# joyce-leesw/Conway-s-GOL-Distributed

Hardware: AMD Instinct MI355X
Metric: cell updates/sec (GCUPS) at 16384² & 65536², 1/2/4/8 MI355X; % HBM roofline (higher is better)
Workload: dtype u32

## Files before the change

### conway-s-gol-distributed_amd/csrc/gol_tile.h

```cpp
#pragma once
#include "gol_device.h"
#if GOL_TOOLS
#include "gol_tile_turn.h"
#else
namespace golk {
template <int SEG, int V>
__device__ __forceinline__ void tile_turn_asm(uint32_t (&v)[SEG][2], uint32_t (&ad)[4], uint32_t ps,
                                              uint32_t ba);
}
#endif

#include <type_traits>

#ifndef GOL_TILE_PAIRS_MAX
#define GOL_TILE_PAIRS_MAX 12
#endif
#ifndef GOL_TURN_VAR
#define GOL_TURN_VAR 4
#endif
#ifndef GOL_TILE_WEST_CARRY
#define GOL_TILE_WEST_CARRY 1
#endif
#ifndef GOL_TILE_RAW
#define GOL_TILE_RAW 0
#endif
#ifndef GOL_TILE_PAIR
#define GOL_TILE_PAIR 0
#endif
#ifndef GOL_TILE_SPIN_LIMIT
#define GOL_TILE_SPIN_LIMIT (1 << 22)
#endif
template <int SEG, int W>
constexpr bool tile_west_carry() { return GOL_TILE_WEST_CARRY && W == 1 && SEG >= 4 && SEG <= 16; }

namespace golk {

constexpr int kTileMaxWaves = 16;
constexpr size_t tile_lds_bytes(int threads, int words)
{
    return (size_t)threads * 4 * 16 * words + 4 * kTileMaxWaves;
}
constexpr int tile_seg_rows(int code) { return code % 100; }
constexpr int tile_seg_words(int code) { return code / 1000 + 1; }
constexpr int tile_slots_pow2(int threads)
{
    int n = 64;
    while (n < threads) n *= 2;
    return n;
}
constexpr size_t tile_count_lds_bytes(int threads)
{
    return 4 * (size_t)kMaxTileTurns * kTileMaxWaves + 4 * (size_t)threads;
}
constexpr size_t tile_lds_bytes_code(int threads, int code)
{
    const int ord = code / 100 % 10;
    return (ord == 8 || ord == 9) && (GOL_TURN_VAR & 4)
               ? tile_lds_bytes(tile_slots_pow2(threads), 1)
           : ord == 3 && GOL_TILE_PAIR ? 2 * tile_lds_bytes(threads, 1)
                                       : tile_lds_bytes(threads, tile_seg_words(code));
}

constexpr uint32_t tile_rcp16(int c) { return (65536u + (uint32_t)c - 1u) / (uint32_t)c; }
constexpr bool tile_rcp16_exact()
{
    for (int c = 3; c <= 64; ++c)
        for (uint32_t l = 0; l < 64; ++l)
            if (((l * tile_rcp16(c)) >> 16) != l / (uint32_t)c) return false;
    return true;
}
static_assert(tile_rcp16_exact(), "lane * ceil(65536 / C) >> 16 == lane / C below 64");

struct TilePos {
    int tw, th, x0, y0, g;
    uint32_t rcp;
};
__device__ __forceinline__ TilePos tile_pos_rect(const StepArgs &a, int tile, int ntx)
{
    const int ty = tile / ntx, tx = tile - ty * ntx;
    const int c = a.tile_w + 2;
    return TilePos{a.tile_w, a.band, tx * a.tile_w, a.row_lo + ty * a.band, 64 / c, tile_rcp16(c)};
}
struct TileLaunch {
    int ntiles, n_main, ntx_main;
    uint32_t inv_ntx;
    int narrow_w, narrow_h;
    int g[2];
    uint32_t rcp[2];
};
__device__ __forceinline__ TilePos tile_pos(const StepArgs &a, const TileLaunch &L, int tile)
{
    if (tile >= L.n_main)
        return TilePos{L.narrow_w, L.narrow_h, L.ntx_main * a.tile_w,
                       a.row_lo + (tile - L.n_main) * L.narrow_h, L.g[1], L.rcp[1]};
    int ty = tile;
    if (L.ntx_main > 1) {
        ty = (int)__umulhi((uint32_t)tile, L.inv_ntx);
        ty -= ty * L.ntx_main > tile ? 1 : 0;
    }
    const int tx = tile - ty * L.ntx_main;
    return TilePos{a.tile_w, a.band, tx * a.tile_w, a.row_lo + ty * a.band, L.g[0], L.rcp[0]};
}

struct RingArgs {
    int tile, ntx;
    uint64_t *u0, *u1;
    unsigned *flags;
    unsigned epoch;
    int turns;
    unsigned *gcount;
    unsigned gbase;
    int ablate;
};
template <int SEG, int ORD, int W, bool PERSIST, bool RING = false, bool CNT = false,
          bool SEAM = false, bool BIG = false>
__device__ __forceinline__ void tile_pass(const uint64_t *__restrict__ in,
                                          uint64_t *__restrict__ out, const StepArgs &a,
                                          int turns, const TilePos &pos,
                                          RingArgs ra = RingArgs{})
{
    constexpr int ND = 2 * W;
    constexpr int NS = 2 * ND;
    static_assert(SEG >= 2, "two edge rows per segment");
    extern __shared__ uint4 xsh[];
    const int nslot = (int)(blockDim.x);
    const int TW = pos.tw, C = TW + 2, G = pos.g;
    const int K = turns, TH = pos.th;
    const int nl = a.nw / W;
    const int y0 = pos.y0;
    const int x0 = pos.x0;
    const int lane = threadIdx.x & 63;
    const int wave = __builtin_amdgcn_readfirstlane((int)(threadIdx.x >> 6));
    const int group = (int)(((uint32_t)lane * pos.rcp) >> 16), col = lane - group * C;
    const bool live = group < G;
    const int nseg = (TH + 2 * K + SEG - 1) / SEG;
    constexpr bool kHalo = ORD == 7;
    static_assert(!kHalo || W == 1, "ORD 7: one word per lane");
    const int seg = !kHalo ? wave * G + group
                           : wave == 0 ? (group == 0 ? 0 : nseg - 1) : (wave - 1) * G + group + 1;
    const bool rev = kHalo && wave == 0 && group == 1;
    const int slot = seg * C + col;

    int gx = x0 - 1 + (live ? col : 0);
    if (nl < C) {
        while (gx < 0) gx += nl;
        while (gx >= nl) gx -= nl;
    } else {
        gx += gx < 0 ? nl : 0;
        gx -= gx >= nl ? nl : 0;
    }
    static_assert(!SEAM || (W == 1 && !PERSIST && !RING && !CNT && ORD != 3 && ORD < 7),
                  "seam launches: plain k_step_tile, one word per lane, no counts");
    [[maybe_unused]] bool seam_tile = false, seam_lane = false;
    [[maybe_unused]] int seam_v = 0;
    [[maybe_unused]] uint32_t seam_d = 0;
    if constexpr (SEAM) {
        const int L = nl - 1;
        seam_tile = x0 == 0 || x0 + TW >= L;
        seam_v = x0 - 1 + (live ? col : 0);
        seam_lane = seam_tile && live && (seam_v < 0 || seam_v >= L);
        const int g2 = seam_lane ? min(seam_second_col(seam_v, L), L) : gx;
        seam_d = (uint32_t)(g2 - gx) * 8u;
    }
    const int M = a.modrows;
    const uint32_t pitch_b = (uint32_t)a.pitch * 8u;
    const uint32_t span = (uint32_t)M * pitch_b;
    int rbase = y0 - K;
    if (rbase < 0) {
        rbase += M;
        while (rbase < 0) rbase += M;
    }
    int r = rbase + (live ? seg : 0) * SEG + (rev ? SEG - 1 : 0);
    if (__builtin_amdgcn_ballot_w64(r >= 2 * M) != 0) {
        while (r >= M) r -= M;
    } else {
        r -= r >= M ? M : 0;
    }
    uint32_t off = (uint32_t)r * pitch_b + (uint32_t)gx * (8u * W);
    [[maybe_unused]] const uint32_t off_first = off;
    const uint32_t lstep = rev ? span - pitch_b : pitch_b;
    const __amdgpu_buffer_rsrc_t rin =
        __builtin_amdgcn_make_buffer_rsrc((void *)in, (short)0, (int)span, kBufFlags);
    static_assert(!BIG || (W == 1 && !PERSIST && !RING && !CNT && !SEAM && ORD != 3 && ORD < 7),
                  "big launches: plain k_step_tile, one word per lane, no seam, no counts");
    [[maybe_unused]] int big_ra = 0, big_rb = 0, big_rs = 0;
    [[maybe_unused]] __amdgpu_buffer_rsrc_t rin_a = rin, rin_b = rin;
    [[maybe_unused]] auto big_rsrc = [](const void *p, uint64_t byte, int rows, uint32_t row_b) {
        const uint64_t ad = (uint64_t)(uintptr_t)p + byte;
        const uint32_t lo = (uint32_t)__builtin_amdgcn_readfirstlane((int)(uint32_t)ad);
        const uint32_t hi = (uint32_t)__builtin_amdgcn_readfirstlane((int)(uint32_t)(ad >> 32));
        const int bytes = __builtin_amdgcn_readfirstlane((int)((uint32_t)rows * row_b));
        return __builtin_amdgcn_make_buffer_rsrc((void *)(uintptr_t)(((uint64_t)hi << 32) | lo),
                                                 (short)0, bytes, kBufFlags);
    };
    if constexpr (BIG) {
        int64_t w0, wa, wb;
        uint64_t ba;
        (void)tile_window(M, a.pitch, y0, K, TH, &w0, &wa, &wb, &ba);
        big_ra = __builtin_amdgcn_readfirstlane((int)wa);
        big_rb = __builtin_amdgcn_readfirstlane((int)wb);
        big_rs = big_ra > 0 ? max(0, min(TH, a.row_hi - y0)) : 0;
        rin_a = big_rsrc(in, ba, big_ra, pitch_b);
        rin_b = big_rsrc(in, 0, big_rb, pitch_b);
    }
    const __amdgpu_buffer_rsrc_t rout =
        BIG ? big_rsrc(out, (uint64_t)(uint32_t)y0 * pitch_b, big_rs, pitch_b)
            : __builtin_amdgcn_make_buffer_rsrc((void *)out, (short)0, (int)span, kBufFlags);

    constexpr int kLoadAux = PERSIST ? 16 : GOL_TILE_LOAD_AUX;
    uint32_t v[SEG][ND];
    auto load_row = [&](int i, uint32_t voff, uint32_t soff) {
        if constexpr (W == 1) {
            const u32x2 w = __builtin_amdgcn_raw_buffer_load_b64(rin, voff, soff, kLoadAux);
            v[i][0] = w.x;
            v[i][1] = w.y;
        } else {
            const u32x4 w = __builtin_amdgcn_raw_buffer_load_b128(rin, voff, soff, kLoadAux);
            v[i][0] = w.x;
            v[i][1] = w.y;
            v[i][2] = w.z;
            v[i][3] = w.w;
        }
    };
    if constexpr (BIG) {
        const int tr0 = (live ? seg : 0) * SEG;
        const uint32_t cb = (uint32_t)gx * 8u;
        const int wlim = big_ra + big_rb;
        if (__builtin_amdgcn_ballot_w64(tr0 + SEG > big_ra) == 0) {
            const uint32_t o = (uint32_t)tr0 * pitch_b + cb;
#pragma unroll
            for (int i = 0; i < SEG; ++i) {
                const u32x2 w = __builtin_amdgcn_raw_buffer_load_b64(rin_a, o, (uint32_t)i * pitch_b, kLoadAux);
                v[i][0] = w.x;
                v[i][1] = w.y;
            }
        } else if (big_rb == 0) {
#pragma unroll
            for (int i = 0; i < SEG; ++i) {
                const uint32_t o = (uint32_t)min(tr0 + i, wlim) * pitch_b + cb;
                const u32x2 w = __builtin_amdgcn_raw_buffer_load_b64(rin_a, o, 0, kLoadAux);
                v[i][0] = w.x;
                v[i][1] = w.y;
            }
        } else {
            constexpr int kBigChunk = 4;
            int tb = tr0;
#pragma unroll
            for (int c0 = 0; c0 < SEG; c0 += kBigChunk) {
                u32x2 pa[kBigChunk], pb[kBigChunk];
#pragma unroll
                for (int j = 0; j < kBigChunk; ++j) {
                    if (c0 + j < SEG) {
                        const int t = min(tb + c0 + j, wlim);
                        const uint32_t oa = (uint32_t)t * pitch_b + cb;
                        const uint32_t ob = (uint32_t)(t - big_ra) * pitch_b + cb;
                        pa[j] = __builtin_amdgcn_raw_buffer_load_b64(rin_a, oa, 0, kLoadAux);
                        pb[j] = __builtin_amdgcn_raw_buffer_load_b64(rin_b, ob, 0, kLoadAux);
                    }
                }
#pragma unroll
                for (int j = 0; j < kBigChunk; ++j) {
                    if (c0 + j < SEG) {
                        const bool second = tb + c0 + j >= big_ra;
                        v[c0 + j][0] = second ? pb[j].x : pa[j].x;
                        v[c0 + j][1] = second ? pb[j].y : pa[j].y;
                    }
                }
                if (c0 + kBigChunk < SEG)
                    asm volatile("" : "+v"(tb) : "v"(v[c0 + kBigChunk - 1][0]),
                                 "v"(v[c0 + kBigChunk - 1][1]));
            }
        }
    } else if (SEAM && seam_tile) {
    } else if (!kHalo && __builtin_amdgcn_ballot_w64(r + SEG > M) == 0) {
#pragma unroll
        for (int i = 0; i < SEG; ++i) load_row(i, off, (uint32_t)i * pitch_b);
    } else {
#pragma unroll
        for (int i = 0; i < SEG; ++i) {
            load_row(i, off, 0);
            off += lstep;
            off = off >= span ? off - span : off;
        }
    }
    if constexpr (SEAM) {
        if (seam_tile) {
            const int L = nl - 1, rb = a.width & 63;
            auto seam_load = [&](auto ODD, auto STEP) {
                constexpr bool odd = decltype(ODD)::value, step = decltype(STEP)::value;
                constexpr int kSeamChunk = 4;
                uint32_t o1 = off_first, o2 = off_first + seam_d;
#pragma unroll
                for (int c0 = 0; c0 < SEG; c0 += kSeamChunk) {
                    u32x2 p[kSeamChunk], t[kSeamChunk];
#pragma unroll
                    for (int j = 0; j < kSeamChunk; ++j) {
                        if (c0 + j < SEG) {
                            const uint32_t so = step ? (uint32_t)(c0 + j) * pitch_b : 0u;
                            p[j] = __builtin_amdgcn_raw_buffer_load_b64(rin, o1, so, kLoadAux);
                            t[j] = __builtin_amdgcn_raw_buffer_load_b64(rin, o2, so, kLoadAux);
                            if constexpr (!step) {
                                o1 += lstep;
                                o1 = o1 >= span ? o1 - span : o1;
                                o2 += lstep;
                                o2 = o2 >= span ? o2 - span : o2;
                            }
                        }
                    }
#pragma unroll
                    for (int j = 0; j < kSeamChunk; ++j) {
                        if (c0 + j < SEG) {
                            const uint64_t pw = ((uint64_t)p[j].y << 32) | p[j].x;
                            const uint64_t sw = ((uint64_t)t[j].y << 32) | t[j].x;
                            const uint64_t w = seam_stitch(pw, sw, seam_v, L, rb, odd, true);
                            v[c0 + j][0] = seam_lane ? (uint32_t)w : p[j].x;
                            v[c0 + j][1] = seam_lane ? (uint32_t)(w >> 32) : p[j].y;
                        }
                    }
                    if (c0 + kSeamChunk < SEG)
                        asm volatile("" : "+v"(o1), "+v"(o2) : "v"(v[c0 + kSeamChunk - 1][0]),
                                     "v"(v[c0 + kSeamChunk - 1][1]));
                }
            };
            using std::false_type;
            using std::true_type;
            const bool nowrap = __builtin_amdgcn_ballot_w64(r + SEG > M) == 0;
            if (rb & 1) {
                if (nowrap) seam_load(true_type{}, true_type{});
                else seam_load(true_type{}, false_type{});
            } else {
                if (nowrap) seam_load(false_type{}, true_type{});
                else seam_load(false_type{}, false_type{});
            }
        }
    }

    auto rsum = [&](const uint32_t (&x)[ND], uint32_t (&s)[NS]) {
        const uint32_t Rt = dpp_from_upper_z(x[0]);
#pragma unroll
        for (int w = 0; w < W; ++w) {
            const uint32_t e = x[2 * w], o = x[2 * w + 1];
            uint32_t wl;
            if constexpr (tile_west_carry<SEG, W>()) {
                const uint64_t m = __builtin_amdgcn_ballot_w64((int)o < 0) << 1;
                uint64_t co;
                asm("v_addc_co_u32_e64 %0, %1, %2, %2, %3" : "=v"(wl), "=&s"(co) : "v"(o), "s"(m));
            } else {
                const uint32_t L = dpp_from_lower_z(x[ND - 1]);
                wl = __builtin_amdgcn_alignbit(o, w == 0 ? L : x[2 * w - 1], 31);
            }
            const uint32_t er = __builtin_amdgcn_alignbit(w == W - 1 ? Rt : x[2 * w + 2], e, 1);
            s[4 * w + 0] = xor3(wl, e, o);
            s[4 * w + 1] = maj(wl, e, o);
            s[4 * w + 2] = xor3(e, o, er);
            s[4 * w + 3] = maj(e, o, er);
        }
    };
    auto rule = [&](const uint32_t (&A)[NS], const uint32_t (&B)[NS], const uint32_t (&Cs)[NS],
                   uint32_t (&x)[ND]) {
        uint32_t n[ND];
#pragma unroll
        for (int d = 0; d < ND; ++d)
            n[d] = life_rule7(A[2 * d], B[2 * d], Cs[2 * d], A[2 * d + 1], B[2 * d + 1],
                              Cs[2 * d + 1], x[d]);
#pragma unroll
        for (int d = 0; d < ND; ++d) x[d] = n[d];
    };
    auto put = [&](uint4 *base, const uint32_t (&S)[NS]) {
#pragma unroll
        for (int q = 0; q < W; ++q)
            base[(size_t)q * nslot * 4] =
                make_uint4(S[4 * q], S[4 * q + 1], S[4 * q + 2], S[4 * q + 3]);
    };
    auto get = [&](const uint4 *base, uint32_t (&S)[NS]) {
#pragma unroll
        for (int q = 0; q < W; ++q) {
            const uint4 u = base[(size_t)q * nslot * 4];
            S[4 * q] = u.x;
            S[4 * q + 1] = u.y;
            S[4 * q + 2] = u.z;
            S[4 * q + 3] = u.w;
        }
    };
    const int nlive = (int)(blockDim.x >> 6) * G * C;
    const int myslot = live ? slot : nlive + wave * (64 - G * C) + (lane - G * C);
    const int s_up = live && seg > 0 ? slot - C : myslot;
    const int s_dn = live && seg + 1 < nseg ? slot + C : myslot;
    const int o_wt = (rev ? (int)nslot : 0) + myslot, o_wb = (rev ? 0 : (int)nslot) + myslot;
    const int o_up = rev ? s_dn : (int)nslot + s_up, o_dn = rev ? (int)nslot + s_up : s_dn;
    constexpr bool kPairs = SEG * W <= GOL_TILE_PAIRS_MAX;
    constexpr bool kRaw = ORD < 4 && W == 1 && SEG <= GOL_TILE_RAW;
    uint4 *const wtop2[2] = {xsh + o_wt, xsh + 2 * nslot + o_wt};
    uint4 *const wbot2[2] = {xsh + o_wb, xsh + 2 * nslot + o_wb};
    const uint4 *const rup2[2] = {xsh + o_up, xsh + 2 * nslot + o_up};
    const uint4 *const rdn2[2] = {xsh + o_dn, xsh + 2 * nslot + o_dn};
    auto wtop = [&](int p, int off) { return kPairs ? wtop2[p] : xsh + off + o_wt; };
    auto wbot = [&](int p, int off) { return kPairs ? wbot2[p] : xsh + off + o_wb; };
    auto rup = [&](int p, int off) { return kPairs ? rup2[p] : (const uint4 *)(xsh + off + o_up); };
    auto rdn = [&](int p, int off) { return kPairs ? rdn2[p] : (const uint4 *)(xsh + off + o_dn); };
    const int wrow0 = __builtin_amdgcn_readfirstlane(
        !kHalo ? wave * G * SEG : wave == 0 ? 0 : ((wave - 1) * G + 1) * SEG);
    const int wrow1 = __builtin_amdgcn_readfirstlane(
        !kHalo ? wrow0 + G * SEG : wave == 0 ? 1 << 30 : wrow0 + G * SEG);
    const int nwaves = (int)(blockDim.x >> 6);
    volatile int *const flag = (volatile int *)(xsh + 4 * (size_t)nslot * W);
    if constexpr (ORD == 4) {
        if (lane == 0) flag[wave] = -1;
        __syncthreads();
    }
    static_assert(!CNT || (W == 1 && !PERSIST && !RING && ORD != 3 && ORD < 7),
                  "counted launches: plain k_step_tile, one word per lane");
    [[maybe_unused]] uint32_t *const csum = (uint32_t *)(xsh + 4 * (size_t)nslot * W) + kTileMaxWaves;
    [[maybe_unused]] int cw_lo = 0, cw_hi = -1;
    static_assert(!CNT || SEG <= 32, "counted launches: one word of row bits per lane");
    [[maybe_unused]] bool cwave = false, cuni = false, cany = false;
    [[maybe_unused]] uint32_t *const crow = csum + kMaxTileTurns * kTileMaxWaves;
    if constexpr (CNT) {
        cw_lo = K / (G * SEG);
        cw_hi = min(nwaves - 1, (K + TH - 1) / (G * SEG));
        cwave = wave >= cw_lo && wave <= cw_hi;
        const int ybase = y0 - K + seg * SEG;
        const int ylo = max(y0, a.cnt_lo), yhi = min(min(y0 + TH, a.row_hi), a.cnt_hi);
        const bool ccol = live && col >= 1 && col <= TW && x0 + col - 1 < nl;
        const int ci_lo = min(max(ylo - ybase, 0), SEG), ci_hi = min(max(yhi - ybase, 0), SEG);
        const int cn = ccol && cwave ? max(ci_hi - ci_lo, 0) : 0;
        crow[threadIdx.x] = cn > 0 ? (~0u >> (32 - cn)) << ci_lo : 0u;
        cany = cn > 0;
        cuni = __builtin_amdgcn_ballot_w64(cn != 0 && cn != SEG) == 0;
    }
    auto bcnt = [](uint32_t x, uint32_t acc) {
        uint32_t r;
        asm("v_bcnt_u32_b32 %0, %1, %2" : "=v"(r) : "v"(x), "v"(acc));
        return r;
    };
    auto bcnt0 = [](uint32_t x) {
        uint32_t r;
        asm("v_bcnt_u32_b32 %0, %1, 0" : "=v"(r) : "v"(x));
        return r;
    };
    auto count_turn = [&](int t) {
        if constexpr (CNT) {
            if (!cwave) return;
            uint32_t acc;
            if (cuni) {
                acc = bcnt(v[0][1], bcnt0(v[0][0]));
#pragma unroll
                for (int i = 1; i < SEG; ++i) acc = bcnt(v[i][1], bcnt(v[i][0], acc));
                acc = cany ? acc : 0u;
            } else {
                uint32_t all = ~0u;
                asm volatile("" : "+v"(all));
                const uint32_t ln = __builtin_amdgcn_mbcnt_hi(all, __builtin_amdgcn_mbcnt_lo(all, 0u));
                const uint32_t rlo = crow[wave * 64 + (int)ln];
                acc = 0;
#pragma unroll
                for (int i = 0; i < SEG; ++i) {
                    const uint32_t m = 0u - ((rlo >> i) & 1u);
                    acc = bcnt(v[i][1] & m, bcnt(v[i][0] & m, acc));
                }
                asm("s_nop 1" : "+v"(acc));
            }
            acc += (uint32_t)__builtin_amdgcn_update_dpp(0, (int)acc, 0x111, 0xf, 0xf, true);
            acc += (uint32_t)__builtin_amdgcn_update_dpp(0, (int)acc, 0x112, 0xf, 0xf, true);
            acc += (uint32_t)__builtin_amdgcn_update_dpp(0, (int)acc, 0x114, 0xf, 0xf, true);
            acc += (uint32_t)__builtin_amdgcn_update_dpp(0, (int)acc, 0x118, 0xf, 0xf, true);
            acc += (uint32_t)__builtin_amdgcn_update_dpp(0, (int)acc, 0x142, 0xa, 0xf, false);
            acc += (uint32_t)__builtin_amdgcn_update_dpp(0, (int)acc, 0x143, 0xc, 0xf, false);
            if (lane == 63) csum[t * kTileMaxWaves + wave] = acc;
        }
    };
    auto publish = [&](int t) {
        if constexpr (ORD == 4) {
            asm volatile("" ::: "memory");
            if (lane == 0) flag[wave] = t;
        }
    };
    auto await_neighbours = [&](int t) {
        if constexpr (ORD == 4) {
            const int up = wave > 0 ? wave - 1 : wave, dn = wave + 1 < nwaves ? wave + 1 : wave;
            for (;;) {
                const int a = __builtin_amdgcn_readfirstlane(flag[up]);
                const int b = __builtin_amdgcn_readfirstlane(flag[dn]);
                if (a >= t && b >= t) break;
                __builtin_amdgcn_s_sleep(1);
            }
            __builtin_amdgcn_fence(__ATOMIC_ACQUIRE, "workgroup");
        }
    };
    auto turn4 = [&](auto P, int poff, int t, int lo_rt) {
        constexpr int p = decltype(P)::value;
        const int lo = ORD == 7 ? lo_rt : 0;
        const int off = poff;
        uint32_t Pw[NS], Q[NS], S1[NS];
        {
            uint32_t F[NS], Lr[NS];
            rsum(v[0], F);
            rsum(v[SEG - 1], Lr);
            put(wtop(p, off), F);
            put(wbot(p, off), Lr);
            if constexpr (ORD == 5 || ORD == 7) __syncthreads();
            else if constexpr (ORD == 4) publish(t);
#pragma unroll
            for (int k = 0; k < NS; ++k) Pw[k] = F[k];
        }
        rsum(v[1], Q);
#pragma unroll
        for (int k = 0; k < NS; ++k) S1[k] = Q[k];
#pragma unroll
        for (int i = 1; i + 1 < SEG; ++i) {
            uint32_t R[NS];
            if (i + 2 == SEG) get(wbot(p, off), R);
            else rsum(v[i + 1], R);
            if (i >= lo) rule(Pw, Q, R, v[i]);
#pragma unroll
            for (int k = 0; k < NS; ++k) {
                Pw[k] = Q[k];
                Q[k] = R[k];
            }
        }
#pragma unroll
        for (int i = 1; i + 1 < SEG; ++i)
#pragma unroll
            for (int d = 0; d < ND; ++d) asm volatile("" : "+v"(v[i][d]));
        if constexpr (ORD == 6) __syncthreads();
        else await_neighbours(t);
        uint32_t U[NS], D[NS], F[NS];
        if (lo == 0) {
            get(rup(p, off), U);
            get(wtop(p, off), F);
            rule(U, F, S1, v[0]);
        }
        get(rdn(p, off), D);
        get(wbot(p, off), F);
        rule(Pw, F, D, v[SEG - 1]);
    };
    auto turn = [&](auto P, int poff, int t) {
        if constexpr (ORD >= 4) {
            turn4(P, poff, t, kHalo && wave == 0 ? min(t + 1, SEG - 2) : 0);
            return;
        }
        constexpr int p = decltype(P)::value;
        const int off = poff;
        uint32_t F[NS], Lr[NS];
        rsum(v[0], F);
        rsum(v[SEG - 1], Lr);
        if constexpr (kRaw) {
            *wtop(p, off) = make_uint4(v[0][0], v[0][1], v[SEG - 1][0], v[SEG - 1][1]);
        } else {
            put(wtop(p, off), F);
            put(wbot(p, off), Lr);
        }
        uint32_t U[NS], D[NS];
        auto get_raw = [&](uint32_t (&Us)[NS], uint32_t (&Ds)[NS]) {
            const uint4 *const base = kPairs ? xsh + 2 * nslot * p : xsh + off;
            const uint2 a = *(reinterpret_cast<const uint2 *>(base + s_up) + 1);
            const uint2 b = *reinterpret_cast<const uint2 *>(base + s_dn);
            const uint32_t ra[ND] = {a.x, a.y}, rb[ND] = {b.x, b.y};
            rsum(ra, Us);
            rsum(rb, Ds);
        };
        if constexpr (ORD < 2 || ORD == 3) {
            if constexpr (ORD != 3) __syncthreads();
            if constexpr (kRaw) {
                get_raw(U, D);
            } else {
                get(rup(p, off), U);
                get(rdn(p, off), D);
            }
        }
        if constexpr (ORD == 0 || ORD == 3) {
            uint32_t A[NS], B[NS];
#pragma unroll
            for (int k = 0; k < NS; ++k) {
                A[k] = U[k];
                B[k] = F[k];
            }
#pragma unroll
            for (int i = 0; i < SEG; ++i) {
                uint32_t Cs[NS];
                if (i + 1 == SEG) {
#pragma unroll
                    for (int k = 0; k < NS; ++k) Cs[k] = D[k];
                } else if (i + 2 == SEG) {
#pragma unroll
                    for (int k = 0; k < NS; ++k) Cs[k] = Lr[k];
                } else {
                    rsum(v[i + 1], Cs);
                }
                rule(A, B, Cs, v[i]);
#pragma unroll
                for (int k = 0; k < NS; ++k) {
                    A[k] = B[k];
                    B[k] = Cs[k];
                }
            }
        } else {
            uint32_t Pw[NS], Q[NS], S1[NS];
#pragma unroll
            for (int k = 0; k < NS; ++k) Pw[k] = F[k];
            if constexpr (SEG >= 3) {
                rsum(v[1], Q);
#pragma unroll
                for (int k = 0; k < NS; ++k) S1[k] = Q[k];
            } else {
#pragma unroll
                for (int k = 0; k < NS; ++k) S1[k] = Q[k] = Lr[k];
            }
#pragma unroll
            for (int i = 1; i + 1 < SEG; ++i) {
                uint32_t R[NS];
                if (i + 2 == SEG) {
#pragma unroll
                    for (int k = 0; k < NS; ++k) R[k] = Lr[k];
                } else {
                    rsum(v[i + 1], R);
                }
                rule(Pw, Q, R, v[i]);
#pragma unroll
                for (int k = 0; k < NS; ++k) {
                    Pw[k] = Q[k];
                    Q[k] = R[k];
                }
            }
            if constexpr (ORD == 2) {
                __syncthreads();
                if constexpr (kRaw) {
                    get_raw(U, D);
                } else {
                    get(rup(p, off), U);
                    get(rdn(p, off), D);
                }
            }
            rule(U, F, S1, v[0]);
            rule(Pw, Lr, D, v[SEG - 1]);
        }
    };
    const int lastrow = 2 * K + TH - 1;
    auto leave = [&](int t) {
        if constexpr (ORD == 4) {
            if (lane == 0) flag[wave] = 0x7fffffff;
        }
    };
    bool gone = false;
    if constexpr (RING) {
        static_assert(PERSIST && W == 1 && ORD != 4 && ORD != 7 && ORD < 8, "K1r: one word per lane");
        const int THv = min(TH, a.row_hi - y0), TWv = min(TW, nl - x0);
        const int nty = (a.row_hi - a.row_lo + TH - 1) / TH;
        const int tile = ra.tile, ntx = ra.ntx, ty = tile / ntx, tx = tile - ty * ntx;
        const int nblocks = (ra.turns + K - 1) / K, kbase = ra.turns / nblocks,
                  kextra = ra.turns % nblocks;
        bool gave_up = false;
        for (int b = 0; b < nblocks; ++b) {
            const int kb = kbase + (b < kextra ? 1 : 0);
            if constexpr (!kPairs) {
                for (int t = 0; t < kb; ++t) turn(std::integral_constant<int, 0>{}, (t & 1) * 2 * nslot, t);
            } else {
                for (int t = 0; t < kb; t += 2) {
                    turn(std::integral_constant<int, 0>{}, 0, t);
                    if (t + 1 == kb) break;
                    turn(std::integral_constant<int, 1>{}, 0, t + 1);
                }
            }
            if (b + 1 == nblocks) break;
            uint64_t *const X = (b & 1) ? ra.u1 : ra.u0;
            const __amdgpu_buffer_rsrc_t rx =
                __builtin_amdgcn_make_buffer_rsrc((void *)X, (short)0, (int)span, kBufFlags);
            int ln = lane, thv = THv, twv = TWv, kk = K;
            uint32_t off0 = off_first;
            asm volatile("" : "+v"(ln), "+v"(off0), "+s"(thv), "+s"(twv), "+s"(kk));
            const int gr = (int)(((uint32_t)ln * pos.rcp) >> 16), cl = ln - gr * C;
            const bool lv = gr < G;
            const int tr0 = (wave * G + gr) * SEG;
            if (lv && cl >= 1 && cl <= twv && !(ra.ablate & 1)) {
                const bool side = cl == 1 || cl == twv;
                uint32_t so = off0;
#pragma unroll
                for (int i = 0; i < SEG; ++i) {
                    const int j = tr0 + i - kk;
                    if (j >= 0 && j < thv && (side || j < kk || j >= thv - kk))
                        buf_store(v[i], rx, so, 0);
                    so += pitch_b;
                    so = so >= span ? so - span : so;
                }
            }
            __builtin_amdgcn_s_waitcnt((7 << 4) | (15 << 8));
            __syncthreads();
            if (threadIdx.x == 0) {
                __hip_atomic_store(ra.flags + tile, ra.epoch + (unsigned)b + 1u, __ATOMIC_RELAXED,
                                   __HIP_MEMORY_SCOPE_AGENT);
            }
            if (ra.gcount && threadIdx.x == 0) {
                __hip_atomic_fetch_add(ra.gcount, 1u, __ATOMIC_RELAXED, __HIP_MEMORY_SCOPE_AGENT);
                const unsigned want = ra.gbase + (unsigned)(b + 1) * (unsigned)(nty * ntx);
                bool seen = false;
                for (int spin = 0; !seen && spin < GOL_TILE_SPIN_LIMIT; ++spin) {
                    const unsigned fv = __hip_atomic_load(ra.gcount, __ATOMIC_RELAXED, __HIP_MEMORY_SCOPE_AGENT);
                    seen = (int)(fv - want) >= 0;
                    if (!seen) __builtin_amdgcn_s_sleep(1);
                }
                gave_up |= !seen;
            }
            if (!ra.gcount && threadIdx.x < 8 && !(ra.ablate & 2)) {
                const int jn = (int)threadIdx.x + (threadIdx.x >= 4 ? 1 : 0);
                const int ny = (ty + jn / 3 - 1 + nty) % nty, nx = (tx + jn % 3 - 1 + ntx) % ntx;
                const unsigned want = ra.epoch + (unsigned)b + 1u;
                const unsigned *f = ra.flags + ny * ntx + nx;
                bool seen = false;
                for (int spin = 0; !seen && spin < GOL_TILE_SPIN_LIMIT; ++spin) {
                    const unsigned fv = __hip_atomic_load(f, __ATOMIC_RELAXED, __HIP_MEMORY_SCOPE_AGENT);
                    seen = (int)(fv - want) >= 0;
                    if (!seen) __builtin_amdgcn_s_sleep(1);
                }
                gave_up |= !seen;
            }
            __atomic_signal_fence(__ATOMIC_SEQ_CST);
            __syncthreads();
            if (lv && !(ra.ablate & 4)) {
                const bool hl = cl == 0 || cl == twv + 1;
                uint32_t lo = off0;
#pragma unroll
                for (int i = 0; i < SEG; ++i) {
                    const int tr = tr0 + i;
                    if (tr < 2 * kk + thv && (hl || tr < kk || tr >= kk + thv)) {
                        const u32x2 w = __builtin_amdgcn_raw_buffer_load_b64(rx, lo, 0, kLoadAux);
                        v[i][0] = w.x;
                        v[i][1] = w.y;
                    }
                    lo += pitch_b;
                    lo = lo >= span ? lo - span : lo;
                }
            }
        }
        if (gave_up && a.err)
            __hip_atomic_store(a.err, kDevErrTileFlag, __ATOMIC_RELAXED, __HIP_MEMORY_SCOPE_SYSTEM);
    } else if constexpr (ORD == 8 || ORD == 9) {
        static_assert(W == 1 && !PERSIST && SEG % 3 == 0, "ORD 8/9: one word per lane, plain launches");
        constexpr int TV = (GOL_TURN_VAR & 6) | (ORD == 9 ? 1 : 0);
        const uint32_t base = (uint32_t)(uintptr_t)(lds_void *)xsh;
        uint32_t ad[4];
        uint32_t ps;
        if constexpr ((TV & 4) != 0) {
            const uint32_t ns = (uint32_t)tile_slots_pow2(nslot);
            ad[0] = base + 16u * (uint32_t)myslot;
            ad[1] = base + 16u * (ns + (uint32_t)myslot);
            ad[2] = base + 16u * (ns + (uint32_t)s_up);
            ad[3] = base + 16u * (uint32_t)s_dn;
            ps = 32u * ns;
        } else {
            ad[0] = base + 64u * (uint32_t)myslot;
            ad[1] = 0u;
            ad[2] = base + 64u * (uint32_t)s_up + 32u;
            ad[3] = base + 64u * (uint32_t)s_dn;
            ps = 16u;
        }
        const int tend = __builtin_amdgcn_readfirstlane(
            max(0, min(K, min(wrow1, lastrow - wrow0 + 1))));
        const uint32_t ba = ORD == 9 ? (uint32_t)((lane + 63) & 63) * 4u : 0u;
        ps = __builtin_amdgcn_readfirstlane(ps);
        for (int t = 0; t < tend; ++t) tile_turn_asm<SEG, TV>(v, ad, ps, ba);
        if (tend < K) return;
        uint32_t all = ~0u;
        asm volatile("" : "+v"(all));
        const int ln = (int)__builtin_amdgcn_mbcnt_hi(all, __builtin_amdgcn_mbcnt_lo(all, 0u));
        const int gr = (int)(((uint32_t)ln * pos.rcp) >> 16), cl = ln - gr * C;
        if (gr >= G || cl < 1 || cl > TW || x0 + cl - 1 >= nl) return;
        const int t0 = (wave * G + gr) * SEG;
        uint32_t so = (uint32_t)(y0 - K + t0) * pitch_b + (uint32_t)(x0 + cl - 1) * 8u;
#pragma unroll
        for (int i = 0; i < SEG; ++i) {
            const int tr = t0 + i;
            if (tr >= K && tr < K + TH && y0 - K + tr < a.row_hi) buf_store(v[i], rout, so, 0);
            so += pitch_b;
        }
        return;
    } else if constexpr (kHalo) {
        static_assert(!kPairs, "ORD 7: long segments");
        for (int t = 0; t < K; ++t) {
            if (!PERSIST && (wrow1 <= t || wrow0 > lastrow - t)) {
                leave(t);
                gone = true;
                break;
            }
            turn(std::integral_constant<int, 0>{}, (t & 1) * 2 * nslot, t);
        }
    } else if constexpr (!kPairs) {
        const int tlast = __builtin_amdgcn_readfirstlane(lastrow - wrow0);
        for (int t = 0; t < K; ++t) {
            if (!PERSIST && (wrow1 <= t || t > tlast)) {
                leave(t);
                gone = true;
                break;
            }
            turn(std::integral_constant<int, 0>{}, (t & 1) * 2 * nslot, t);
            count_turn(t);
        }
    } else {
        for (int t = 0; t < K; t += 2) {
            if (!PERSIST && (wrow1 <= t || wrow0 > lastrow - t)) {
                leave(t);
                gone = true;
                break;
            }
            turn(std::integral_constant<int, 0>{}, 0, t);
            count_turn(t);
            if (t + 1 == K) break;
            if (!PERSIST && (wrow1 <= t + 1 || wrow0 > lastrow - t - 1)) {
                leave(t + 1);
                gone = true;
                break;
            }
            turn(std::integral_constant<int, 1>{}, 0, t + 1);
            count_turn(t + 1);
        }
    }
    if (!PERSIST && gone) return;
    if constexpr (CNT) {
        __syncthreads();
        uint32_t all = ~0u;
        asm volatile("" : "+v"(all));
        const int ln = (int)__builtin_amdgcn_mbcnt_hi(all, __builtin_amdgcn_mbcnt_lo(all, 0u));
        if (wave == cw_lo && ln < K) {
            uint32_t s = 0;
            for (int w = cw_lo; w <= cw_hi; ++w) s += csum[ln * kTileMaxWaves + w];
            if (s)
                atomicAdd(a.counts + (size_t)ln * kShards + (blockIdx.x & (kShards - 1)),
                          (unsigned long long)s);
        }
    }
    if (gone) return;
    auto store_row = [&](int i, uint32_t voff, uint32_t soff) {
        if constexpr (W == 1 && GOL_TILE_STORE_AUX != 0) {
            const u32x2 d = {v[i][0], v[i][1]};
            __builtin_amdgcn_raw_buffer_store_b64(d, rout, voff, soff, GOL_TILE_STORE_AUX);
        } else {
            buf_store(v[i], rout, voff, soff);
        }
    };
    if constexpr (!kHalo) {
        uint32_t all = ~0u;
        asm volatile("" : "+v"(all));
        const int sl = (int)__builtin_amdgcn_mbcnt_hi(all, __builtin_amdgcn_mbcnt_lo(all, 0u));
        const int sg = (int)(((uint32_t)sl * pos.rcp) >> 16), sc = sl - sg * C;
        const bool scol = sg < G && sc >= 1 && sc <= TW && x0 + sc - 1 < nl;
        const int t0 = (wave * G + sg) * SEG;
        const int top = min(K + TH, a.row_hi - (y0 - K));
        const int lo = min(max(K - t0, 0), SEG), hi = min(max(top - t0, 0), SEG);
        uint32_t so = (uint32_t)(BIG ? t0 - K : y0 - K + t0) * pitch_b + (uint32_t)(x0 + sc - 1) * (8u * W);
        if constexpr (SEAM) {
            const int L = nl - 1;
            if (x0 <= L && x0 + TW > L) {
                const int rb = a.width & 63;
                const bool lastc = x0 + sc - 1 == L;
                const uint32_t me = lastc ? ~0u >> (32 - ((rb + 1) >> 1)) : ~0u;
                const uint32_t mo = lastc ? (1u << (rb >> 1)) - 1u : ~0u;
#pragma unroll
                for (int i = 0; i < SEG; ++i) {
                    v[i][0] &= me;
                    v[i][1] &= mo;
                }
            }
        }
        if (__builtin_amdgcn_ballot_w64(scol && (lo > 0 || hi < SEG)) == 0) {
            if (scol) {
#pragma unroll
                for (int i = 0; i < SEG; ++i) store_row(i, so, (uint32_t)i * pitch_b);
            }
            return;
        }
        if (!scol || hi <= lo) return;
#pragma unroll
        for (int i = 0; i < SEG; ++i) {
            if (i >= lo && i < hi) store_row(i, so, 0);
            so += pitch_b;
        }
        return;
    }
    if (!live || col < 1 || col > TW || x0 + col - 1 >= nl) return;
    const int t0 = seg * SEG + (rev ? SEG - 1 : 0);
    const int dr = rev ? -1 : 1;
    const uint32_t sstep = rev ? 0u - pitch_b : pitch_b;
    uint32_t so = (uint32_t)(y0 - K + t0) * pitch_b + (uint32_t)(x0 + col - 1) * (8u * W);
#pragma unroll
    for (int i = 0; i < SEG; ++i) {
        const int tr = t0 + dr * i;
        if (tr >= K && tr < K + TH && y0 - K + tr < a.row_hi) {
            if constexpr (W == 1 && GOL_TILE_STORE_AUX != 0)
                buf_store_aux<GOL_TILE_STORE_AUX>(v[i], rout, so);
            else
                buf_store(v[i], rout, so, 0);
        }
        so += sstep;
    }
}

template <int SEG>
__device__ __forceinline__ void tile_pass_pair(const uint64_t *__restrict__ in,
                                               uint64_t *__restrict__ out, const StepArgs &a,
                                               int turns, int tileA, int tileB, bool storeB,
                                               int ntx)
{
    constexpr int ND = 2, NS = 4;
    static_assert(SEG >= 2 && SEG <= 8, "ORD 3: short segments");
    extern __shared__ uint4 xsh[];
    const int nslot = (int)blockDim.x;
    const int TW = a.tile_w, C = TW + 2, G = 64 / C;
    const int K = turns, TH = a.band;
    const int nl = a.nw;
    const int lane = threadIdx.x & 63;
    const int wave = __builtin_amdgcn_readfirstlane((int)(threadIdx.x >> 6));
    const int group = lane / C, col = lane - group * C;
    const bool live = group < G;
    const int nseg = (TH + 2 * K + SEG - 1) / SEG;
    const int seg = wave * G + group;
    const int slot = seg * C + col;
    const int M = a.modrows;
    const uint32_t pitch_b = (uint32_t)a.pitch * 8u;
    const uint32_t span = (uint32_t)M * pitch_b;
    const __amdgpu_buffer_rsrc_t rin =
        __builtin_amdgcn_make_buffer_rsrc((void *)in, (short)0, (int)span, kBufFlags);
    const __amdgpu_buffer_rsrc_t rout =
        __builtin_amdgcn_make_buffer_rsrc((void *)out, (short)0, (int)span, kBufFlags);
    const int tiles[2] = {tileA, tileB};
    uint32_t v[2][SEG][ND];
    int y0s[2], x0s[2];
#pragma unroll
    for (int X = 0; X < 2; ++X) {
        const int ty = tiles[X] / ntx, tx = tiles[X] - ty * ntx;
        y0s[X] = a.row_lo + ty * TH;
        x0s[X] = tx * TW;
        int gx = x0s[X] - 1 + (live ? col : 0);
        while (gx < 0) gx += nl;
        while (gx >= nl) gx -= nl;
        int r = y0s[X] - K + (live ? seg : 0) * SEG;
        while (r < 0) r += M;
        while (r >= M) r -= M;
        uint32_t off = (uint32_t)r * pitch_b + (uint32_t)gx * 8u;
#pragma unroll
        for (int i = 0; i < SEG; ++i) {
            const u32x2 w = __builtin_amdgcn_raw_buffer_load_b64(rin, off, 0, 0);
            v[X][i][0] = w.x;
            v[X][i][1] = w.y;
            off += pitch_b;
            off = off >= span ? off - span : off;
        }
    }
    auto rsum = [&](const uint32_t (&x)[ND], uint32_t (&s)[NS]) {
        const uint32_t Rt = dpp_from_upper_z(x[0]);
        const uint32_t e = x[0], o = x[1];
        uint32_t wl;
        if constexpr (tile_west_carry<SEG, 1>()) {
            const uint64_t m = __builtin_amdgcn_ballot_w64((int)o < 0) << 1;
            uint64_t co;
            asm("v_addc_co_u32_e64 %0, %1, %2, %2, %3" : "=v"(wl), "=&s"(co) : "v"(o), "s"(m));
        } else {
            wl = __builtin_amdgcn_alignbit(o, dpp_from_lower_z(o), 31);
        }
        const uint32_t er = __builtin_amdgcn_alignbit(Rt, e, 1);
        s[0] = xor3(wl, e, o);
        s[1] = maj(wl, e, o);
        s[2] = xor3(e, o, er);
        s[3] = maj(e, o, er);
    };
    auto rule = [&](const uint32_t (&A)[NS], const uint32_t (&B)[NS], const uint32_t (&Cs)[NS],
                    uint32_t (&x)[ND]) {
        uint32_t n[ND];
#pragma unroll
        for (int d = 0; d < ND; ++d)
            n[d] = life_rule7(A[2 * d], B[2 * d], Cs[2 * d], A[2 * d + 1], B[2 * d + 1],
                              Cs[2 * d + 1], x[d]);
#pragma unroll
        for (int d = 0; d < ND; ++d) x[d] = n[d];
    };
    auto put = [&](uint4 *p, const uint32_t (&S)[NS]) { *p = make_uint4(S[0], S[1], S[2], S[3]); };
    auto get = [&](const uint4 *p, uint32_t (&S)[NS]) {
        const uint4 u = *p;
        S[0] = u.x;
        S[1] = u.y;
        S[2] = u.z;
        S[3] = u.w;
    };
    const int nlive = (int)(blockDim.x >> 6) * G * C;
    const int myslot = live ? slot : nlive + wave * (64 - G * C) + (lane - G * C);
    const int s_up = live && seg > 0 ? slot - C : myslot;
    const int s_dn = live && seg + 1 < nseg ? slot + C : myslot;
    auto at = [&](int X, int p, int bt, int sl) { return xsh + ((X * 2 + p) * 2 + bt) * nslot + sl; };
    uint32_t F[2][NS], Lr[2][NS], S1[2][NS], Pl[2][NS];
    auto h1 = [&](auto XX, auto PP) {
        constexpr int X = decltype(XX)::value, p = decltype(PP)::value;
        rsum(v[X][0], F[X]);
        rsum(v[X][SEG - 1], Lr[X]);
        put(at(X, p, 0, myslot), F[X]);
        put(at(X, p, 1, myslot), Lr[X]);
        uint32_t Pw[NS], Q[NS];
#pragma unroll
        for (int k = 0; k < NS; ++k) Pw[k] = F[X][k];
        if constexpr (SEG >= 3) {
            rsum(v[X][1], Q);
        } else {
#pragma unroll
            for (int k = 0; k < NS; ++k) Q[k] = Lr[X][k];
        }
#pragma unroll
        for (int k = 0; k < NS; ++k) S1[X][k] = Q[k];
#pragma unroll
        for (int i = 1; i + 1 < SEG; ++i) {
            uint32_t R[NS];
            if (i + 2 == SEG) {
#pragma unroll
                for (int k = 0; k < NS; ++k) R[k] = Lr[X][k];
            } else {
                rsum(v[X][i + 1], R);
            }
            rule(Pw, Q, R, v[X][i]);
#pragma unroll
            for (int k = 0; k < NS; ++k) {
                Pw[k] = Q[k];
                Q[k] = R[k];
            }
        }
#pragma unroll
        for (int k = 0; k < NS; ++k) Pl[X][k] = Pw[k];
    };
    auto h2 = [&](auto XX, auto PP) {
        constexpr int X = decltype(XX)::value, p = decltype(PP)::value;
        uint32_t U[NS], D[NS];
        get(at(X, p, 1, s_up), U);
        get(at(X, p, 0, s_dn), D);
        rule(U, F[X], S1[X], v[X][0]);
        rule(Pl[X], Lr[X], D, v[X][SEG - 1]);
    };
    using I0 = std::integral_constant<int, 0>;
    using I1 = std::integral_constant<int, 1>;
    const int lastrow = 2 * K + TH - 1;
    const int wrow0 = wave * G * SEG, wrow1 = wrow0 + G * SEG;
    auto leaves = [&](int t) { return wrow1 <= t || wrow0 > lastrow - t; };
    h1(I0{}, I0{});
    __syncthreads();
    bool gone = false;
    for (int t = 0; t < K; t += 2) {
        if (leaves(t)) {
            gone = true;
            break;
        }
        h2(I0{}, I0{});
        h1(I1{}, I0{});
        __syncthreads();
        h2(I1{}, I0{});
        if (t + 1 == K) break;
        h1(I0{}, I1{});
        __syncthreads();
        if (leaves(t + 1)) {
            gone = true;
            break;
        }
        h2(I0{}, I1{});
        h1(I1{}, I1{});
        __syncthreads();
        h2(I1{}, I1{});
        if (t + 2 == K) break;
        h1(I0{}, I0{});
        __syncthreads();
    }
    if (gone || !live || col < 1 || col > TW) return;
    const int t0 = seg * SEG;
#pragma unroll
    for (int X = 0; X < 2; ++X) {
        if (X == 1 && !storeB) break;
        if (x0s[X] + col - 1 >= nl) continue;
        uint32_t so = (uint32_t)(y0s[X] - K + t0) * pitch_b + (uint32_t)(x0s[X] + col - 1) * 8u;
#pragma unroll
        for (int i = 0; i < SEG; ++i) {
            const int tr = t0 + i;
            if (tr >= K && tr < K + TH && y0s[X] - K + tr < a.row_hi) buf_store(v[X][i], rout, so, 0);
            so += pitch_b;
        }
    }
}

__device__ __forceinline__ int tile_of_block(int ntiles)
{
    const int per = (ntiles + 7) / 8;
    return (int)(blockIdx.x % 8) * per + (int)(blockIdx.x / 8);
}

template <int SEG, int ORD, int W>
__global__ __launch_bounds__(1024, (ORD == 7 ? 6 : 1)) void k_step_tile(const uint64_t *__restrict__ in,
                                                     uint64_t *__restrict__ out, StepArgs a,
                                                     int turns, TileLaunch L)
{
    const int tile = tile_of_block(L.ntiles);
    if (tile >= L.ntiles) return;
    tile_pass<SEG, ORD, W, false>(in, out, a, turns, tile_pos(a, L, tile));
}

template <int SEG, int ORD>
__global__ __launch_bounds__(1024, (SEG <= 16 ? 8 : 6)) void k_step_tile_seam(const uint64_t *__restrict__ in,
                                                            uint64_t *__restrict__ out, StepArgs a,
                                                            int turns, TileLaunch L)
{
    const int tile = tile_of_block(L.ntiles);
    if (tile >= L.ntiles) return;
    tile_pass<SEG, ORD, 1, false, false, false, true>(in, out, a, turns, tile_pos(a, L, tile));
}

template <int SEG, int ORD>
__global__ __launch_bounds__(1024, (SEG <= 16 ? 8 : 6)) void k_step_tile_big(
    const uint64_t *__restrict__ in, uint64_t *__restrict__ out, StepArgs a, int turns, TileLaunch L)
{
    const int tile = tile_of_block(L.ntiles);
    if (tile >= L.ntiles) return;
    tile_pass<SEG, ORD, 1, false, false, false, false, true>(in, out, a, turns, tile_pos(a, L, tile));
}

template <int SEG, int ORD, int W>
__global__ __launch_bounds__(1024, 1) void k_step_tile_cnt(const uint64_t *__restrict__ in,
                                                           uint64_t *__restrict__ out, StepArgs a,
                                                           int turns, TileLaunch L)
{
    const int tile = tile_of_block(L.ntiles);
    if (tile >= L.ntiles) return;
    tile_pass<SEG, ORD, W, false, false, true>(in, out, a, turns, tile_pos(a, L, tile));
}

template <int SEG>
__global__ __launch_bounds__(1024, 1) void k_step_tile_pair(const uint64_t *__restrict__ in,
                                                            uint64_t *__restrict__ out, StepArgs a,
                                                            int turns, int ntx, int ntiles)
{
    const int npairs = (ntiles + 1) / 2;
    const int pair = tile_of_block(npairs);
    if (pair >= npairs) return;
    const int tA = 2 * pair, tB = 2 * pair + 1 < ntiles ? 2 * pair + 1 : 2 * pair;
    tile_pass_pair<SEG>(in, out, a, turns, tA, tB, 2 * pair + 1 < ntiles, ntx);
}

template <int SEG, int ORD, int W>
__global__ __launch_bounds__(1024, 1) void k_tile_persist(
    const uint64_t *__restrict__ in, uint64_t *__restrict__ out, uint64_t *u0, uint64_t *u1,
    StepArgs a, int turns, int K, int ntx, int ntiles, unsigned *flags, unsigned epoch)
{
    const int tile = tile_of_block(ntiles);
    if (tile >= ntiles) return;
    const int nty = ntiles / ntx, ty = tile / ntx, tx = tile - ty * ntx;
    const int nblocks = (turns + K - 1) / K, base = turns / nblocks, extra = turns % nblocks;
    bool gave_up = false;
    for (int b = 0; b < nblocks; ++b) {
        const int k = base + (b < extra ? 1 : 0);
        if (b > 0) {
            if (threadIdx.x < 8) {
                const int j = (int)threadIdx.x + (threadIdx.x >= 4 ? 1 : 0);
                const int dy = j / 3 - 1, dx = j % 3 - 1;
                const int ny = (ty + dy + nty) % nty, nx = (tx + dx + ntx) % ntx;
                const unsigned want = epoch + (unsigned)b;
                unsigned *f = flags + ny * ntx + nx;
                bool seen = false;
                for (int spin = 0; !seen && spin < GOL_TILE_SPIN_LIMIT; ++spin) {
                    const unsigned v =
                        __hip_atomic_load(f, __ATOMIC_RELAXED, __HIP_MEMORY_SCOPE_AGENT);
                    seen = (int)(v - want) >= 0;
                    if (!seen) __builtin_amdgcn_s_sleep(2);
                }
                gave_up |= !seen;
            }
            __atomic_signal_fence(__ATOMIC_SEQ_CST);
            __syncthreads();
        }
        const uint64_t *src = b == 0 ? in : ((b & 1) ? u0 : u1);
        uint64_t *dst = b + 1 == nblocks ? out : ((b & 1) ? u1 : u0);
        tile_pass<SEG, ORD, W, true>(src, dst, a, k, tile_pos_rect(a, tile, ntx));
        if (b + 1 == nblocks) break;
        __builtin_amdgcn_s_waitcnt((7 << 4) | (15 << 8));
        __syncthreads();
        if (threadIdx.x == 0)
            __hip_atomic_store(flags + tile, epoch + (unsigned)b + 1u, __ATOMIC_RELAXED,
                               __HIP_MEMORY_SCOPE_AGENT);
    }
    if (gave_up && a.err)
        __hip_atomic_store(a.err, kDevErrTileFlag, __ATOMIC_RELAXED, __HIP_MEMORY_SCOPE_SYSTEM);
}


template <int SEG, int ORD>
__global__ __launch_bounds__(1024, 1) void k_tile_ring(
    const uint64_t *__restrict__ in, uint64_t *__restrict__ out, uint64_t *u0, uint64_t *u1,
    StepArgs a, int turns, int K, int ntx, int ntiles, unsigned *flags, unsigned epoch,
    unsigned *gcount, unsigned gbase, int ablate)
{
    const int tile = tile_of_block(ntiles);
    if (tile >= ntiles) return;
    tile_pass<SEG, ORD, 1, true, true>(in, out, a, K, tile_pos_rect(a, tile, ntx),
                                       RingArgs{tile, ntx, u0, u1, flags, epoch, turns, gcount, gbase,
                                                ablate});
}

template <int SEG, int ORD, int W>
__global__ __launch_bounds__(1024, (SEG >= 20 ? 6 : 8)) void k_tile_stream(
    const uint64_t *__restrict__ in, uint64_t *__restrict__ out, uint64_t *u0, uint64_t *u1,
    StepArgs a, int turns, int K, int ntx, int ntiles, unsigned *flags, unsigned epoch,
    unsigned *counter, unsigned base)
{
    __shared__ unsigned next_item;
    const int nty = ntiles / ntx;
    const int nblocks = (turns + K - 1) / K, kbase = turns / nblocks, extra = turns % nblocks;
    const unsigned nitems = (unsigned)nblocks * (unsigned)ntiles;
    bool gave_up = false;
    if (threadIdx.x == 0)
        next_item = __hip_atomic_fetch_add(counter, 1u, __ATOMIC_RELAXED, __HIP_MEMORY_SCOPE_AGENT) - base;
    __syncthreads();
    for (;;) {
        const unsigned item = next_item;
        __syncthreads();
        if (item >= nitems) break;
        unsigned nxt = 0;
        if (threadIdx.x == 0)
            nxt = __hip_atomic_fetch_add(counter, 1u, __ATOMIC_RELAXED, __HIP_MEMORY_SCOPE_AGENT) - base;
        const int b = (int)(item / (unsigned)ntiles), j = (int)(item % (unsigned)ntiles);
        const int ty = (j / ntx + 2 * b) % nty, tx = j % ntx;
        const int tile = ty * ntx + tx;
        const int k = kbase + (b < extra ? 1 : 0);
        if (b > 0) {
            if (threadIdx.x < 9) {
                const int jj = (int)threadIdx.x;
                const int dy = jj / 3 - 1, dx = jj % 3 - 1;
                const int ny = (ty + dy + nty) % nty, nx = (tx + dx + ntx) % ntx;
                const unsigned want = epoch + (unsigned)b;
                unsigned *f = flags + ny * ntx + nx;
                bool seen = false;
                for (int spin = 0; !seen && spin < GOL_TILE_SPIN_LIMIT; ++spin) {
                    const unsigned v =
                        __hip_atomic_load(f, __ATOMIC_RELAXED, __HIP_MEMORY_SCOPE_AGENT);
                    seen = (int)(v - want) >= 0;
                    if (!seen) __builtin_amdgcn_s_sleep(2);
                }
                gave_up |= !seen;
            }
            __atomic_signal_fence(__ATOMIC_SEQ_CST);
            if (threadIdx.x < 64) {
                __builtin_amdgcn_fence(__ATOMIC_ACQUIRE, "agent");
                asm volatile("s_waitcnt vmcnt(0)" ::: "memory");
            }
            __syncthreads();
        }
        const uint64_t *src = b == 0 ? in : ((b & 1) ? u0 : u1);
        uint64_t *dst = b + 1 == nblocks ? out : ((b & 1) ? u1 : u0);
        StepArgs aa = a;
        asm volatile("" : "+s"(aa.tile_w), "+s"(aa.band), "+s"(aa.nw), "+s"(aa.pitch),
                     "+s"(aa.modrows));
        tile_pass<SEG, ORD, W, true>(src, dst, aa, k, tile_pos_rect(aa, tile, ntx));
        if (b + 1 < nblocks) {
            __builtin_amdgcn_s_waitcnt((7 << 4) | (15 << 8));
            __syncthreads();
            if (threadIdx.x == 0) {
                __builtin_amdgcn_fence(__ATOMIC_RELEASE, "agent");
                asm volatile("s_waitcnt vmcnt(0)" ::: "memory");
                __hip_atomic_store(flags + tile, epoch + (unsigned)b + 1u, __ATOMIC_RELAXED,
                                   __HIP_MEMORY_SCOPE_AGENT);
            }
        }
        if (threadIdx.x == 0) next_item = nxt;
        __syncthreads();
    }
    if (gave_up && a.err)
        __hip_atomic_store(a.err, kDevErrTileFlag, __ATOMIC_RELAXED, __HIP_MEMORY_SCOPE_SYSTEM);
}

}
```

Before: 137,500.

## Pin tile turn registers to fixed VGPRs with parity-aware allocation for SEG16 ORD5

Adds a specialized turn path for the ORD 5, single-word, SEG 16 tile configuration that pins cell rows, row sums and temporaries to explicit VGPR numbers via inline-asm register constraints. It swizzles sum halves so operands land in registers of matching parity, and reorders the rule computation to fit that plan. The goal is to stop the compiler's register allocator from inserting moves or bank conflicts in the unrolled hot loop. In exchange it adds rigid hand register assignment that may fight the compiler, limit scheduling freedom, or raise register pressure.

```diff
diff --git a/conway-s-gol-distributed_amd/csrc/gol_tile.h b/conway-s-gol-distributed_amd/csrc/gol_tile.h
--- a/conway-s-gol-distributed_amd/csrc/gol_tile.h
+++ b/conway-s-gol-distributed_amd/csrc/gol_tile.h
@@ -32,8 +32,45 @@
 #endif
 template <int SEG, int W>
 constexpr bool tile_west_carry() { return GOL_TILE_WEST_CARRY && W == 1 && SEG >= 4 && SEG <= 16; }
+#ifndef GOL_TILE_PARITY_PINS
+#define GOL_TILE_PARITY_PINS 1
+#endif
 
 namespace golk {
+
+template <int N>
+__device__ __forceinline__ void vpin(uint32_t &x);
+#define GOL_VPIN(N)                                                                               \
+    template <>                                                                                   \
+    __device__ __forceinline__ void vpin<N>(uint32_t &x) { asm("" : "+{v" #N "}"(x)); }
+#define GOL_VPIN8(A, B, C, D, E, F, G, H)                                                         \
+    GOL_VPIN(A) GOL_VPIN(B) GOL_VPIN(C) GOL_VPIN(D) GOL_VPIN(E) GOL_VPIN(F) GOL_VPIN(G) GOL_VPIN(H)
+GOL_VPIN8(0, 1, 2, 3, 4, 5, 6, 7)
+GOL_VPIN8(8, 9, 10, 11, 12, 13, 14, 15)
+GOL_VPIN8(16, 17, 18, 19, 20, 21, 22, 23)
+GOL_VPIN8(24, 25, 26, 27, 28, 29, 30, 31)
+GOL_VPIN8(32, 33, 34, 35, 36, 37, 38, 39)
+GOL_VPIN8(40, 41, 42, 43, 44, 45, 46, 47)
+GOL_VPIN8(48, 49, 50, 51, 52, 53, 54, 55)
+GOL_VPIN8(56, 57, 58, 59, 60, 61, 62, 63)
+GOL_VPIN8(64, 65, 66, 67, 68, 69, 70, 71)
+GOL_VPIN8(72, 73, 74, 75, 76, 77, 78, 79)
+#undef GOL_VPIN8
+#undef GOL_VPIN
+
+constexpr int tile_pin_cell(int i, int d) { return 2 * i + d; }
+constexpr int tile_pin_sum(int seg, int j, int k)
+{
+    const int base = 2 * seg + (j == 1 ? 16 : (j & 1) * 8 + ((j >> 1) & 1) * 4);
+    return base + ((j & 1) ? k ^ 1 : k);
+}
+constexpr int tile_pin_tmp(int seg, int d, int t) { return 2 * seg + 20 + 2 * t + (d ^ 1); }
+template <int SEG, int ORD, int W, bool PERSIST, bool RING, bool CNT, bool SEAM, bool BIG>
+constexpr bool tile_parity_pins()
+{
+    return GOL_TILE_PARITY_PINS && ORD == 5 && W == 1 && !PERSIST && !RING && !SEAM && !BIG &&
+           SEG == 16;
+}
 
 constexpr int kTileMaxWaves = 16;
 constexpr size_t tile_lds_bytes(int threads, int words)
@@ -122,6 +159,9 @@
     constexpr int ND = 2 * W;
     constexpr int NS = 2 * ND;
     static_assert(SEG >= 2, "two edge rows per segment");
+    constexpr bool kPins = tile_parity_pins<SEG, ORD, W, PERSIST, RING, CNT, SEAM, BIG>();
+    static_assert(!kPins || (SEG % 2 == 0 && SEG >= 4 && 2 * SEG + 24 <= 80),
+                  "pinned turns: an even segment (the plan's last row is odd), registers below v80");
     extern __shared__ uint4 xsh[];
     const int nslot = (int)(blockDim.x);
     const int TW = pos.tw, C = TW + 2, G = pos.g;
@@ -534,7 +574,124 @@
         get(wbot(p, off), F);
         rule(Pw, F, D, v[SEG - 1]);
     };
+    [[maybe_unused]] auto turn4p = [&](auto P, int poff) {
+        if constexpr (kPins) {
+            constexpr int p = decltype(P)::value;
+            const int off = poff;
+            auto swz = [](uint32_t (&S)[NS]) {
+                const uint32_t s0 = S[0], s2 = S[2];
+                S[0] = S[1];
+                S[1] = s0;
+                S[2] = S[3];
+                S[3] = s2;
+            };
+            auto rsum_p = [&](auto J, uint32_t (&S)[NS]) {
+                constexpr int j = decltype(J)::value;
+                rsum(v[j], S);
+                vpin<tile_pin_sum(SEG, j, 0)>(S[0]);
+                vpin<tile_pin_sum(SEG, j, 1)>(S[1]);
+                vpin<tile_pin_sum(SEG, j, 2)>(S[2]);
+                vpin<tile_pin_sum(SEG, j, 3)>(S[3]);
+            };
+            auto rule_d = [&](auto I, auto Dw, const uint32_t (&A)[NS], const uint32_t (&B)[NS],
+                              const uint32_t (&Cs)[NS]) {
+                constexpr int i = decltype(I)::value, d = decltype(Dw)::value;
+                constexpr int jd = i == 0 ? 1 : i - 1;
+                constexpr int r0 = tile_pin_sum(SEG, jd, 2 * d), r1 = tile_pin_sum(SEG, jd, 2 * d + 1);
+                constexpr int rt = tile_pin_tmp(SEG, d, 0);
+                const uint32_t Cc = v[i][d];
+                const uint32_t lm = maj(A[2 * d], B[2 * d], Cs[2 * d]);
+                uint32_t lx = bitop3<0x7e>(A[2 * d], B[2 * d], Cs[2 * d]);
+                uint32_t hm, hx;
+                if constexpr (i == 2) {
+                    vpin<rt>(lx);
+                    hm = maj(A[2 * d + 1], B[2 * d + 1], Cs[2 * d + 1]);
+                    vpin<tile_pin_tmp(SEG, d, 1)>(hm);
+                    const uint32_t g1 = bitop3<0x16>(lm, lx, Cc);
+                    const uint32_t g2 = bitop3<0x86>(hm, Cc, g1);
+                    hx = xor3(A[2 * d + 1], B[2 * d + 1], Cs[2 * d + 1]);
+                    vpin<tile_pin_cell(i, d)>(hx);
+                    uint32_t n = bitop3<0x82>(lx, hx, g2);
+                    vpin<tile_pin_cell(i, d)>(n);
+                    return n;
+                } else if constexpr ((r1 & 1) == d) {
+                    vpin<r0>(lx);
+                    hm = maj(A[2 * d + 1], B[2 * d + 1], Cs[2 * d + 1]);
+                    vpin<rt>(hm);
+                    hx = xor3(A[2 * d + 1], B[2 * d + 1], Cs[2 * d + 1]);
+                    vpin<r1>(hx);
+                } else {
+                    vpin<rt>(lx);
+                    hx = xor3(A[2 * d + 1], B[2 * d + 1], Cs[2 * d + 1]);
+                    vpin<r0>(hx);
+                    hm = maj(A[2 * d + 1], B[2 * d + 1], Cs[2 * d + 1]);
+                    vpin<r1>(hm);
+                }
+                const uint32_t g1 = bitop3<0x16>(lm, lx, Cc);
+                const uint32_t g2 = bitop3<0x86>(hm, Cc, g1);
+                uint32_t n = bitop3<0x82>(lx, hx, g2);
+                vpin<tile_pin_cell(i, d)>(n);
+                return n;
+            };
+            auto rule_p = [&](auto I, const uint32_t (&A)[NS], const uint32_t (&B)[NS],
+                              const uint32_t (&Cs)[NS]) {
+                constexpr int i = decltype(I)::value;
+                const uint32_t n0 = rule_d(I, std::integral_constant<int, 0>{}, A, B, Cs);
+                const uint32_t n1 = rule_d(I, std::integral_constant<int, 1>{}, A, B, Cs);
+                v[i][0] = n0;
+                v[i][1] = n1;
+            };
+            uint32_t Pw[NS], Q[NS], S1[NS];
+            {
+                uint32_t F[NS], Lr[NS];
+                rsum_p(std::integral_constant<int, 0>{}, F);
+                rsum_p(std::integral_constant<int, SEG - 1>{}, Lr);
+                put(wtop(p, off), F);
+                swz(Lr);
+                put(wbot(p, off), Lr);
+                __syncthreads();
+#pragma unroll
+                for (int k = 0; k < NS; ++k) Pw[k] = F[k];
+            }
+            rsum_p(std::integral_constant<int, 1>{}, Q);
+#pragma unroll
+            for (int k = 0; k < NS; ++k) S1[k] = Q[k];
+            unroll_seq(std::make_integer_sequence<int, SEG - 2>{}, [&](auto I0) {
+                constexpr int i = decltype(I0)::value + 1;
+                uint32_t R[NS];
+                if constexpr (i + 2 == SEG) {
+                    get(wbot(p, off), R);
+                    swz(R);
+                } else {
+                    rsum_p(std::integral_constant<int, i + 1>{}, R);
+                }
+                rule_p(std::integral_constant<int, i>{}, Pw, Q, R);
+#pragma unroll
+                for (int k = 0; k < NS; ++k) {
+                    Pw[k] = Q[k];
+                    Q[k] = R[k];
+                }
+            });
+#pragma unroll
+            for (int i = 1; i + 1 < SEG; ++i)
+#pragma unroll
+                for (int d = 0; d < ND; ++d) asm volatile("" : "+v"(v[i][d]));
+            uint32_t U[NS], D[NS], F[NS];
+            get(rup(p, off), U);
+            swz(U);
+            get(wtop(p, off), F);
+            rule_p(std::integral_constant<int, 0>{}, U, F, S1);
+            get(rdn(p, off), D);
+            get(wbot(p, off), F);
+            swz(F);
+            rule_p(std::integral_constant<int, SEG - 1>{}, Pw, F, D);
+        }
+    };
     auto turn = [&](auto P, int poff, int t) {
+        if constexpr (kPins) {
+            turn4p(P, poff);
+            return;
+        }
         if constexpr (ORD >= 4) {
             turn4(P, poff, t, kHalo && wave == 0 ? min(t + 1, SEG - 2) : 0);
             return;
@@ -635,6 +792,13 @@
             rule(Pw, Lr, D, v[SEG - 1]);
         }
     };
+    if constexpr (kPins) {
+        unroll_seq(std::make_integer_sequence<int, SEG>{}, [&](auto I) {
+            constexpr int i = decltype(I)::value;
+            vpin<tile_pin_cell(i, 0)>(v[i][0]);
+            vpin<tile_pin_cell(i, 1)>(v[i][1]);
+        });
+    }
     const int lastrow = 2 * K + TH - 1;
     auto leave = [&](int t) {
         if constexpr (ORD == 4) {
```

New measurement: 142,100, median of 6. 3.3% higher.
